# keyber/Single-Image-Super-Resolution

Hardware: AMD Instinct MI355X
Metric: HR patches/sec (x2 generator fwd+bwd, LR 96x96 -> SR 192x192) (higher is better)
Workload: dtype f32; 1 GPU; SRGAN x2 generator (16 blocks, 64 features, spectral norm) fwd+bwd+Adam with bicubic LR degradation and pixel-MSE x10, per-GPU batch 16 HR 192x192 patches (LR 96x96 -> SR 192x192): the north star's headline. BASELINE.json's metric string "96^2 crops, x4" is configs.cfg3 of this line. Single build: fp32.; per_gpu_batch=16, hr=192, lr=96, parallelism=dp1, hip_graph=True

## Files before the change

### single-image-super-resolution_amd/csrc/conv_trunk_f32.hip

```cpp
#include "sisr_dev.h"
#include "sisr_bf16_stage.h"
#include "sisr_instr.h"

typedef unsigned cf_u32x4 __attribute__((ext_vector_type(4)));

#include <type_traits>

#define CF_TH 8
#define CF_TW 16
#define CF_IH (CF_TH + 2)
#define CF_IW (CF_TW + 2)
#define CF_NPIX (CF_IH * CF_IW)
#define CF_PSF 36
#define CF_HALO_BYTES (CF_NPIX * CF_PSF * 4)
#define CF_WROW 36
#define CF_WCHUNK_BYTES (9 * 32 * CF_WROW * 4)
#define CF_ITEMS ((CF_NPIX * 8 + 255) / 256)
#define CF_THREADS 512
#define CF_KROWP 100
#define CF_PS 33

SISR_TRACE_BUFFER(sisr_cftrace, 512, 128)
#define CFT(k) SISR_TRACE_STAMP(sisr_cftrace, threadIdx.x == 0, blockIdx.x, k, 64, wall_clock64())
#define CFTP(k) SISR_TRACE_STAMP(sisr_cftrace, threadIdx.x == 256, blockIdx.x, 64 + (k), 128, wall_clock64())
SISR_TRACE_BUFFER(sisr_cfclk, 512, 2)
#define CFTC(k) SISR_TRACE_STAMP(sisr_cfclk, threadIdx.x == 0, blockIdx.x, (k) - 60, 2, clock64())

struct CTrunkF32Args {
    const float *x1, *x2;
    float* x_out;
    BnFinArgs fin;
    const float *pa, *pb, *pd, *ps, *pt;
    const float* slope_p; float slope;
    const float* wpk;
    const void* wimg;
    const float* bias;
    const float* res;
    float* y;
    float *stat_part, *cnt_part;
    const float *bnb_x, *bnb_scale, *bnb_shift, *bnb_mean, *bnb_invstd, *bnb_slope_p;
    float bnb_slope; int bnb_act;
    float* bnb_part;
    int N, H, W;
    int tiles_x, per_img, total, streams;
    uint32_t m_tiles_x, m_per_img;
    int glog, cout_pad, shuffle;
    int xsc, xph;
};

__device__ __forceinline__ __amdgpu_buffer_rsrc_t cf_rsrc(const void* p, unsigned bytes) {
    return __builtin_amdgcn_make_buffer_rsrc(const_cast<void*>(p), 0, (int)bytes, 0x00020000);
}

__device__ __forceinline__ void cf_split2(float v0, float v1, unsigned& hw, unsigned& lw) {
    const f32x2 v = {v0, v1};
    hw = __builtin_bit_cast(unsigned, __builtin_convertvector(v, bf16x2));
    const f32x2 r = {v0 - __uint_as_float(hw << 16), v1 - __uint_as_float(hw & 0xFFFF0000u)};
    lw = __builtin_bit_cast(unsigned, __builtin_convertvector(r, bf16x2));
}

template <int PRO, bool SPLIT>
__global__ void __launch_bounds__(CF_THREADS, 2) conv_trunk_f32_kernel(const CTrunkF32Args a) {
    extern __shared__ __attribute__((aligned(16))) unsigned char lds[];
    unsigned char* halo0 = lds + 2 * CF_WCHUNK_BYTES;
    float* red = reinterpret_cast<float*>(halo0 + 2 * CF_HALO_BYTES);

    const int tid = threadIdx.x, lane = tid & 63;
    const int wave = __builtin_amdgcn_readfirstlane(tid >> 6);
    const bool consumer = wave < 4;
    const int l31 = lane & 31, kk = lane >> 5;
    const bool xcd = (a.streams & 7) == 0;
    const int hc = xcd ? (blockIdx.x >> 3) & ((1 << a.glog) - 1) : blockIdx.x & ((1 << a.glog) - 1);
    const int stream = xcd ? (blockIdx.x & 7) | ((blockIdx.x >> (3 + a.glog)) << 3) : blockIdx.x >> a.glog;
    const unsigned tbytes = (unsigned)a.N * (unsigned)a.H * (unsigned)a.W * 256u;
    constexpr bool TWO = PRO == SISR_PRO_BNBWD || PRO == SISR_PRO_BNACT_BWD || PRO == SISR_PRO_RES_AFFINE || PRO == SISR_PRO_ACT_BWD;
    constexpr bool SUM = PRO == SISR_PRO_RES_AFFINE;
    auto tile_coords = [&](int T, int& n, int& ty, int& tx) {
        n = fdiv(T, a.m_per_img);
        const int rem = T - n * a.per_img;
        ty = fdiv(rem, a.m_tiles_x);
        tx = rem - ty * a.tiles_x;
    };

    CFT(0);
    CFTC(60);
    float* kfin = red + 4 * 32 * 3;
    const bool fin = (PRO == SISR_PRO_AFFINE_ACT || PRO == SISR_PRO_RES_AFFINE) && a.fin.stat != nullptr;
    if (fin) bn_finalize_in_kernel(a.fin, reinterpret_cast<double*>(lds), kfin, blockIdx.x == 0);
    auto fill_weights = [&]() {
        float* wl = reinterpret_cast<float*>(lds);
        if (a.wimg != nullptr) {
            constexpr int UNITS = 2 * 9 * 32 * CF_WROW / 4;
            constexpr int W_IT16 = (UNITS + CF_THREADS - 1) / CF_THREADS;
            const cf_u32x4* src = reinterpret_cast<const cf_u32x4*>(a.wimg) + hc * UNITS;
            cf_u32x4 wv16[W_IT16];
#pragma unroll
            for (int it = 0; it < W_IT16; ++it) {
                const int u = tid + it * CF_THREADS;
                wv16[it] = u < UNITS ? src[u] : cf_u32x4{0u, 0u, 0u, 0u};
            }
#pragma unroll
            for (int it = 0; it < W_IT16; ++it) {
                const int u = tid + it * CF_THREADS;
                if (u < UNITS) reinterpret_cast<cf_u32x4*>(wl)[u] = wv16[it];
            }
            return;
        }
        constexpr int W_IT = 2 * 9 * 32 * 32 / CF_THREADS;
        float wv[W_IT];
#pragma unroll
        for (int it = 0; it < W_IT; ++it) {
            const int e = tid + it * CF_THREADS;
            const int ci = e & 31, s = (e >> 5) % 3, t2 = (e >> 5) / 3;
            const int co = t2 & 31, qr = t2 >> 5;
            wv[it] = a.wpk[((int64_t)qr * a.cout_pad + 32 * hc + co) * CF_KROWP + s * CF_PS + ci];
        }
#pragma unroll
        for (int it = 0; it < W_IT; ++it) {
            const int e = tid + it * CF_THREADS;
            const int ci = e & 31, s = (e >> 5) % 3, t2 = (e >> 5) / 3;
            const int co = t2 & 31, qr = t2 >> 5;
            const int q = qr / 3, r = qr - 3 * q;
            if constexpr (SPLIT) {
                const float vo = __shfl_xor(wv[it], 1);
                const bool odd = ci & 1;
                unsigned hw, lw;
                cf_split2(odd ? vo : wv[it], odd ? wv[it] : vo, hw, lw);
                reinterpret_cast<unsigned*>(wl)[((q * 9 + r * 3 + s) * 32 + co) * CF_WROW + (odd ? 16 : 0) + (ci >> 1)] = odd ? lw : hw;
            } else {
                wl[((q * 9 + r * 3 + s) * 32 + co) * CF_WROW + ci] = wv[it];
            }
        }
    };

    const int n_mine = stream < a.total ? (a.total - stream + a.streams - 1) / a.streams : 0;
    const int n_stages = 2 * n_mine;

    if (!consumer) {
        const int pt = tid & 255, quad = tid & 7, m0 = pt >> 3;
        const int tiles_y = a.per_img / a.tiles_x;
        const float slope = PRO != SISR_PRO_NONE ? (a.slope_p ? a.slope_p[0] : a.slope) : 1.f;
        f32x4 ka[2], kb[2], kd[2], ks[2], kt[2];
        int rel[CF_ITEMS];
        unsigned flags = 0;
#pragma unroll
        for (int k = 0; k < CF_ITEMS; ++k) {
            const int px = m0 + 32 * k;
            const int py = px / CF_IW, pxx = px - py * CF_IW;
            rel[k] = ((py - 1) * a.xsc * a.xsc * a.W + (pxx - 1) * a.xsc) * 256 + quad * 16;
            const unsigned f = (py == 0 ? 1u : 0u) | (py == CF_IH - 1 ? 2u : 0u) | (pxx == 0 ? 4u : 0u) | (pxx == CF_IW - 1 ? 8u : 0u) |
                               (px >= CF_NPIX ? 16u : 0u);
            flags |= f << (5 * k);
            asm volatile("" : "+v"(rel[k]));
        }
        const bool last_beyond = m0 + 32 * (CF_ITEMS - 1) >= CF_NPIX;
        const int ldso = SPLIT ? m0 * CF_PSF * 4 + quad * 8 : (m0 * CF_PSF + quad * 4) * 4;
        const bool easy_slope = slope >= 0.f && slope <= 1.f;

        struct Stage { f32x4 s1[CF_ITEMS], s2[CF_ITEMS]; unsigned bad, origin; bool edge; };
        Stage stA, stB;
        auto issue = [&](int j, Stage& st) {
            const int T = stream + (j >> 1) * a.streams, q = j & 1;
            const unsigned xbytes = (unsigned)(a.xsc * a.xsc) * tbytes;
            const __amdgpu_buffer_rsrc_t r1 = cf_rsrc(a.x1, xbytes), r2 = cf_rsrc(TWO ? a.x2 : a.x1, xbytes);
            int n, ty, tx;
            tile_coords(T, n, ty, tx);
            const unsigned origin = (unsigned)(((n * a.xsc * a.H + a.xsc * ty * CF_TH + (a.xph >> 1)) * a.xsc * a.W + a.xsc * tx * CF_TW + (a.xph & 1)) * 256 + q * 128);
            const unsigned e = (ty == 0 ? 1u : 0u) | (ty == tiles_y - 1 ? 2u : 0u) | (tx == 0 ? 4u : 0u) | (tx == a.tiles_x - 1 ? 8u : 0u);
            st.edge = e != 0u;
            st.bad = flags & ((e | 16u) * 0x02108421u);
            st.origin = origin;
#pragma unroll
            for (int k = 0; k < CF_ITEMS; ++k) {
                const unsigned voff = origin + (unsigned)rel[k];
                st.s1[k] = __builtin_bit_cast(f32x4, __builtin_amdgcn_raw_buffer_load_b128(r1, voff, 0, 0));
                if (TWO) st.s2[k] = __builtin_bit_cast(f32x4, __builtin_amdgcn_raw_buffer_load_b128(r2, voff, 0, 0));
            }
        };
        auto commit_t = [&](auto easy_, auto edge_, int j, const Stage& st) {
            constexpr int EASY = decltype(easy_)::value;
            constexpr bool EDGE = decltype(edge_)::value;
            const int q = j & 1;
            float* img = reinterpret_cast<float*>(halo0 + (j & 1) * CF_HALO_BYTES + ldso);
            const f32x4 qa = q ? ka[1] : ka[0], qb = q ? kb[1] : kb[0], qd = q ? kd[1] : kd[0], qs = q ? ks[1] : ks[0], qt = q ? kt[1] : kt[0];
            const __amdgpu_buffer_rsrc_t ro = cf_rsrc(SUM ? a.x_out : a.x1, tbytes);
#pragma unroll
            for (int k = 0; k < CF_ITEMS; ++k) {
                if (k == CF_ITEMS - 1 && last_beyond) break;
                const bool ok = !EDGE || ((st.bad >> (5 * k)) & 31u) == 0u;
                auto value = [&](int c) {
                    const float v = st.s1[k][c];
                    if (PRO == SISR_PRO_NONE) return v;
                    if (PRO == SISR_PRO_ACT) return lrelu_t<EASY>(v, slope);
                    if (PRO == SISR_PRO_AFFINE_ACT) return lrelu_t<EASY>(qa[c] * v + qd[c], slope);
                    if (SUM) return lrelu_t<EASY>(v, slope) + (qa[c] * st.s2[k][c] + qd[c]);
                    if (PRO == SISR_PRO_ACT_BWD) return st.s2[k][c] > 0.f ? v : slope * v;
                    const float bx = st.s2[k][c];
                    float g = v;
                    if (PRO == SISR_PRO_BNACT_BWD) g = qs[c] * bx + qt[c] > 0.f ? v : slope * v;
                    return qa[c] * g + qb[c] * bx + qd[c];
                };
                const f32x4 osum = {value(0), value(1), value(2), value(3)};
                const f32x4 zero4 = {0.f, 0.f, 0.f, 0.f};
                if constexpr (SPLIT) {
                    typedef unsigned cf_u32x2 __attribute__((ext_vector_type(2)));
                    unsigned h0, l0, h1, l1;
                    cf_split2(osum[0], osum[1], h0, l0);
                    cf_split2(osum[2], osum[3], h1, l1);
                    const cf_u32x2 hw = {h0, h1}, lw = {l0, l1};
                    const cf_u32x2 z2 = {0u, 0u};
                    *reinterpret_cast<cf_u32x2*>(img + k * 32 * CF_PSF) = ok ? hw : z2;
                    *reinterpret_cast<cf_u32x2*>(img + k * 32 * CF_PSF + 16) = ok ? lw : z2;
                } else
                *reinterpret_cast<f32x4*>(img + k * 32 * CF_PSF) = ok ? osum : zero4;
                if (SUM && hc == 0 && ((flags >> (5 * k)) & 31u) == 0u)
                    __builtin_amdgcn_raw_buffer_store_b128(__builtin_bit_cast(cf_u32x4, osum), ro, st.origin + (unsigned)rel[k], 0, 0);
            }
        };
        auto commit = [&](int j, const Stage& st) {
            using T1 = std::integral_constant<int, 1>; using T0 = std::integral_constant<int, 0>;
            constexpr bool HAS_ACT = PRO == SISR_PRO_ACT || PRO == SISR_PRO_AFFINE_ACT || SUM;
            if (!HAS_ACT || easy_slope) {
                if (st.edge) commit_t(T1{}, std::true_type{}, j, st); else commit_t(T1{}, std::false_type{}, j, st);
            } else {
                if (st.edge) commit_t(T0{}, std::true_type{}, j, st); else commit_t(T0{}, std::false_type{}, j, st);
            }
        };

        issue(0, stA);
        issue(1, stB);
#pragma unroll
        for (int q = 0; q < 2; ++q)
#pragma unroll
            for (int j = 0; j < 4; ++j) {
                const int c = q * 32 + quad * 4 + j;
                constexpr bool AFF = PRO == SISR_PRO_AFFINE_ACT || (TWO && PRO != SISR_PRO_ACT_BWD);
                ka[q][j] = fin ? kfin[c] : AFF ? a.pa[c] : 1.f;
                kd[q][j] = fin ? kfin[64 + c] : AFF ? a.pd[c] : 0.f;
                kb[q][j] = (TWO && !SUM && PRO != SISR_PRO_ACT_BWD) ? a.pb[c] : 0.f;
                ks[q][j] = PRO == SISR_PRO_BNACT_BWD ? a.ps[c] : 0.f;
                kt[q][j] = PRO == SISR_PRO_BNACT_BWD ? a.pt[c] : 0.f;
            }
        fill_weights();
        __syncthreads();
        if (n_stages > 0) commit(0, stA);
        __syncthreads();
        int j = 0;
        while (j < n_stages) {
            CFTP(4 + 6 * j);
            issue(j + 2, stA);
            CFTP(5 + 6 * j);
            if (j + 1 < n_stages) commit(j + 1, stB);
            CFTP(8 + 6 * j);
            __syncthreads();
            CFTP(9 + 6 * j);
            if (++j >= n_stages) break;
            CFTP(4 + 6 * j);
            issue(j + 2, stB);
            CFTP(5 + 6 * j);
            if (j + 1 < n_stages) commit(j + 1, stA);
            CFTP(8 + 6 * j);
            __syncthreads();
            CFTP(9 + 6 * j);
            ++j;
        }
    } else {
        const int co = a.shuffle ? 32 * (hc & 1) + l31 : 32 * hc + l31;
        const int ph = hc >> 1;
        const int abase = SPLIT ? ((2 * wave + (l31 >> 4)) * CF_IW + (l31 & 15)) * CF_PSF * 4 + 16 * kk
                                : (((2 * wave + (l31 >> 4)) * CF_IW + (l31 & 15)) * CF_PSF + 16 * kk) * 4;
        const int bbase = SPLIT ? l31 * CF_WROW * 4 + 16 * kk : (l31 * CF_WROW + 16 * kk) * 4;
        const float bv = a.bias != nullptr ? a.bias[a.shuffle ? co * 4 + ph : co] : 0.f;
        float st_shift = 0.f, st_s1 = 0.f, st_s2 = 0.f;
        int st_n = 0;
        const __amdgpu_buffer_rsrc_t ry = cf_rsrc(a.y, a.shuffle ? 4u * tbytes : tbytes), rr = cf_rsrc(a.res != nullptr ? a.res : a.y, tbytes);
        f32x16 acc;
        f32x16 rv, xv;
        const bool has_x = (PRO == SISR_PRO_BNBWD || PRO == SISR_PRO_BNACT_BWD) && a.bnb_part != nullptr;
        const __amdgpu_buffer_rsrc_t rxb = cf_rsrc(has_x ? a.bnb_x : a.y, tbytes);
        float b_sc = 0.f, b_sf = 0.f, b_mu = 0.f, b_is = 0.f, b_slope = 1.f;
        float rs1 = 0.f, rs2 = 0.f, rsl = 0.f;
        if (has_x) {
            b_sc = a.bnb_scale[co]; b_sf = a.bnb_shift[co]; b_mu = a.bnb_mean[co]; b_is = a.bnb_invstd[co];
            b_slope = a.bnb_slope_p ? a.bnb_slope_p[0] : a.bnb_slope;
        }
        fill_weights();
        __syncthreads();
        __syncthreads();
        constexpr bool BWD = TWO && !SUM;
        const bool has_res = BWD && a.res != nullptr;
        const bool x_act = has_x && a.bnb_act != 0;
        const bool do_stat = !BWD && a.stat_part != nullptr;
        const bool shuf = !TWO && a.shuffle != 0;
        const int vl_plain = co * 4 + kk * 4 * 256, vl_shuf = co * 4 + kk * 4 * 512;
        const int tiles_y = fdiv(a.per_img, a.m_tiles_x);
        const int dn = fdiv(a.streams, a.m_per_img), drem = a.streams - dn * a.per_img;
        const int dty = fdiv(drem, a.m_tiles_x), dtx = drem - dty * a.tiles_x;
        int n, ty, tx;
        tile_coords(stream, n, ty, tx);
        auto mma = [&](auto q_c, auto&& mid) {
            constexpr int Q = decltype(q_c)::value;
            const unsigned char* ab = halo0 + Q * CF_HALO_BYTES + abase;
            const unsigned char* bb = lds + Q * CF_WCHUNK_BYTES + bbase;
            if constexpr (SPLIT) {
                bf16x8 ah[9][2], al[9][2], bh[9][2], bl[9][2];
                auto fetch_s = [&](int t) {
                    const unsigned char* pa = ab + ((t / 3) * CF_IW + (t % 3)) * CF_PSF * 4;
                    const unsigned char* pb = bb + t * 32 * CF_WROW * 4;
#pragma unroll
                    for (int ks = 0; ks < 2; ++ks) {
                        ah[t][ks] = *reinterpret_cast<const bf16x8*>(pa + 32 * ks);
                        bh[t][ks] = *reinterpret_cast<const bf16x8*>(pb + 32 * ks);
                        al[t][ks] = *reinterpret_cast<const bf16x8*>(pa + 64 + 32 * ks);
                        bl[t][ks] = *reinterpret_cast<const bf16x8*>(pb + 64 + 32 * ks);
                    }
                };
                fetch_s(0);
                fetch_s(1);
                mid();
                __builtin_amdgcn_sched_barrier(0);
#pragma unroll
                for (int t = 0; t < 9; ++t) {
                    if (t + 2 < 9) fetch_s(t + 2);
#pragma unroll
                    for (int ks = 0; ks < 2; ++ks) {
                        acc = __builtin_amdgcn_mfma_f32_32x32x16_bf16(al[t][ks], bh[t][ks], acc, 0, 0, 0);
                        acc = __builtin_amdgcn_mfma_f32_32x32x16_bf16(ah[t][ks], bl[t][ks], acc, 0, 0, 0);
                        acc = __builtin_amdgcn_mfma_f32_32x32x16_bf16(ah[t][ks], bh[t][ks], acc, 0, 0, 0);
                    }
                    __builtin_amdgcn_sched_barrier(0);
                }
            } else {
                f32x4 af[18][2], bf[18][2];
                auto fetch = [&](int u) {
                    const int t = u >> 1, s0 = 8 * (u & 1);
#pragma unroll
                    for (int v = 0; v < 2; ++v) {
                        af[u][v] = *reinterpret_cast<const f32x4*>(ab + (((t / 3) * CF_IW + (t % 3)) * CF_PSF + s0 + 4 * v) * 4);
                        bf[u][v] = *reinterpret_cast<const f32x4*>(bb + ((t * 32) * CF_WROW + s0 + 4 * v) * 4);
                    }
                };
                fetch(0);
                fetch(1);
                __builtin_amdgcn_sched_barrier(0);
                mid();
                __builtin_amdgcn_sched_barrier(0);
#pragma unroll
                for (int u = 0; u < 18; ++u) {
                    if (u + 2 < 18) fetch(u + 2);
#pragma unroll
                    for (int s = 0; s < 8; ++s) acc = __builtin_amdgcn_mfma_f32_32x32x2f32(af[u][s >> 2][s & 3], bf[u][s >> 2][s & 3], acc, 0, 0, 0);
                    if (u + 2 < 18) __builtin_amdgcn_sched_group_barrier(0x100, 4, 0);
                    __builtin_amdgcn_sched_group_barrier(0x008, 8, 0);
                }
            }
        };
        auto each_value = [&](auto ocol_c, unsigned sb, int orow, auto&& f) {
            constexpr int OCOL = decltype(ocol_c)::value;
            constexpr bool FAR = 11 * OCOL > 4095;
            const unsigned s0 = sb, s1 = sb + (unsigned)orow, s0f = s0 + 8u * OCOL, s1f = s1 + 8u * OCOL;
#pragma unroll
            for (int i = 0; i < 16; ++i) {
                const bool hi = (i >> 2) & 1;
                const unsigned so = (i >> 3) ? (FAR && hi ? s1f : s1) : (FAR && hi ? s0f : s0);
                f(i, (unsigned)(((FAR ? 0 : 8 * hi) + (i & 3)) * OCOL), so);
            }
        };
        using OcolPlain = std::integral_constant<int, 256>;
        using OcolShuf = std::integral_constant<int, 512>;
        for (int t = 0; t < n_mine; ++t) {
            const unsigned sb = (unsigned)(((n * a.H + ty * CF_TH + 2 * wave) * a.W + tx * CF_TW) * 256);
            int vlp = vl_plain, vls = vl_shuf;
            asm volatile("" : "+v"(vlp), "+v"(vls));
            CFT(4 + 12 * t);
            mma(std::integral_constant<int, 0>{}, [&]() {
#pragma unroll
                for (int i = 0; i < 16; ++i) acc[i] = bv;
            });
            CFT(6 + 12 * t);
            CFT(8 + 12 * t);
            __syncthreads();
            CFT(9 + 12 * t);
            CFT(10 + 12 * t);
            mma(std::integral_constant<int, 1>{}, [&]() {
                if (has_res)
                    each_value(OcolPlain{}, sb, a.W * 256, [&](int i, unsigned imm, unsigned so) {
                        rv[i] = __builtin_bit_cast(float, __builtin_amdgcn_raw_buffer_load_b32(rr, (unsigned)vlp + imm, so, 0));
                    });
                if (has_x)
                    each_value(OcolPlain{}, sb, a.W * 256, [&](int i, unsigned imm, unsigned so) {
                        xv[i] = __builtin_bit_cast(float, __builtin_amdgcn_raw_buffer_load_b32(rxb, (unsigned)vlp + imm, so, 0));
                    });
            });
            CFT(12 + 12 * t);
            if (has_res) {
#pragma unroll
                for (int i = 0; i < 16; ++i) acc[i] += rv[i];
            }
            if (has_x) {
                if (x_act) {
#pragma unroll
                    for (int i = 0; i < 16; ++i) {
                        float gv = acc[i];
                        const float z = b_sc * xv[i] + b_sf;
                        const bool neg = !(z > 0.f);
                        rsl += neg ? gv * z : 0.f;
                        gv = neg ? gv * b_slope : gv;
                        rs1 += gv;
                        rs2 += gv * ((xv[i] - b_mu) * b_is);
                    }
                } else {
#pragma unroll
                    for (int i = 0; i < 16; ++i) {
                        rs1 += acc[i];
                        rs2 += acc[i] * ((xv[i] - b_mu) * b_is);
                    }
                }
            }
            if (do_stat) {
                if (st_n == 0) {
                    float s = 0.f;
#pragma unroll
                    for (int i = 0; i < 16; ++i) s += acc[i];
                    st_shift = s * (1.f / 16.f);
                }
#pragma unroll
                for (int i = 0; i < 16; ++i) {
                    const float dv = acc[i] - st_shift;
                    st_s1 += dv;
                    st_s2 += dv * dv;
                }
                st_n += 16;
            }
            if (shuf) {
                const unsigned sbs = (unsigned)(((n * 2 * a.H + 2 * (ty * CF_TH + 2 * wave) + (ph >> 1)) * 2 * a.W + 2 * tx * CF_TW + (ph & 1)) * 256);
                each_value(OcolShuf{}, sbs, 4 * a.W * 256, [&](int i, unsigned imm, unsigned so) {
                    __builtin_amdgcn_raw_buffer_store_b32(__builtin_bit_cast(unsigned, (float)acc[i]), ry, (unsigned)vls + imm, so, 0);
                });
            } else {
                each_value(OcolPlain{}, sb, a.W * 256, [&](int i, unsigned imm, unsigned so) {
                    __builtin_amdgcn_raw_buffer_store_b32(__builtin_bit_cast(unsigned, (float)acc[i]), ry, (unsigned)vlp + imm, so, 0);
                });
            }
            CFT(14 + 12 * t);
            __syncthreads();
            CFT(15 + 12 * t);
            tx += dtx;
            if (tx >= a.tiles_x) { tx -= a.tiles_x; ++ty; }
            ty += dty;
            if (ty >= tiles_y) { ty -= tiles_y; ++n; }
            n += dn;
        }
        CFT(3);

        if (a.stat_part != nullptr) {
            float nn = (float)st_n, mu = 0.f, m2 = 0.f;
            if (st_n > 0) {
                const float m1 = st_s1 / nn;
                mu = st_shift + m1;
                m2 = st_s2 - st_s1 * m1;
            }
            const float nb = __shfl_xor(nn, 32), mub = __shfl_xor(mu, 32), m2b = __shfl_xor(m2, 32);
            const float nt = nn + nb;
            if (nt > 0.f) { const float dl = mub - mu, f = nb / nt; mu += dl * f; m2 += m2b + dl * dl * nn * f; }
            nn = nt;
            if (kk == 0) { float* r = red + (wave * 32 + l31) * 3; r[0] = nn; r[1] = mu; r[2] = m2; }
        }
        if (has_x) {
            rs1 += __shfl_xor(rs1, 32);
            rs2 += __shfl_xor(rs2, 32);
            rsl += __shfl_xor(rsl, 32);
            if (kk == 0) { float* r = red + (wave * 32 + l31) * 3; r[0] = rs1; r[1] = rs2; r[2] = rsl; }
        }
    }
    if (a.bnb_part != nullptr) {
        __syncthreads();
        float* wk = a.bnb_part + (int64_t)blockIdx.x * 129;
        if (tid < 64) {
            const int c = tid & 31;
            const bool mine = (tid >> 5) == hc;
            float s1 = 0.f, s2 = 0.f;
            if (mine) {
                s1 = (red[c * 3] + red[(32 + c) * 3]) + (red[(64 + c) * 3] + red[(96 + c) * 3]);
                s2 = (red[c * 3 + 1] + red[(32 + c) * 3 + 1]) + (red[(64 + c) * 3 + 1] + red[(96 + c) * 3 + 1]);
            }
            wk[tid] = s1;
            wk[64 + tid] = s2;
        }
        if (tid == 64) {
            float sl = 0.f;
            for (int i = 0; i < 128; ++i) sl += red[i * 3 + 2];
            wk[128] = sl;
        }
    }
    if (a.stat_part != nullptr) {
        __syncthreads();
        if (tid < 32) {
            float nn = red[tid * 3], mm = red[tid * 3 + 1], qq = red[tid * 3 + 2];
#pragma unroll
            for (int w = 1; w < 4; ++w) {
                const float* r1 = red + (w * 32 + tid) * 3;
                const float nb = r1[0], nt = nn + nb;
                if (nt > 0.f) { const float dl = r1[1] - mm, f = nb / nt; mm += dl * f; qq += r1[2] + dl * dl * nn * f; }
                nn = nt;
            }
            float* sp = a.stat_part + (int64_t)stream * 128 + 32 * hc + tid;
            sp[0] = mm;
            sp[64] = qq;
            if (tid == 0 && hc == 0) a.cnt_part[stream] = nn;
        }
    }
    CFT(63);
    CFTC(61);
}

#include "sisr_trunk_host.h"
static const SisrTrunkKind CF_KIND = {CF_TH, CF_TW, false, 256};

int sisr_conv2d_trunk_f32_streams(const SisrConvDesc* d) {
    return sisr_equal_shares(d->N * (d->H / CF_TH) * (d->W / CF_TW), sisr_cu_slots() / (d->Cout == 256 ? 8 : 2));
}

extern "C" int sisr_conv2d_trunk_f32_eligible(const SisrConvDesc* d) {
    if (!d || sisr_switch_off("SISR_TRUNK")) return 0;
    if (sisr_switch_off("SISR_TRUNK_F32CONV")) return 0;
    if (!sisr_switch_off("SISR_TRUNK_UP") && d->Cin == 256 && d->Cout == 64 && d->KH == 3 && d->KW == 3 && d->stride == 1 && d->pad_y == 1 && d->pad_x == 1 &&
        d->x_mode == SISR_X_NHWC_UNSHUFFLE2 && d->pro_mode == SISR_PRO_ACT_BWD && d->x2 && d->y_mode == SISR_Y_NHWC && !d->x_bf16 && !d->y_bf16 &&
        !d->res_bf16 && d->Ho == d->H && d->Wo == d->W && !(d->H % CF_TH) && !(d->W % CF_TW) && d->y_sy == 1 && d->y_sx == 1 && !d->y_oy && !d->y_ox &&
        d->y_H == d->Ho && d->y_W == d->Wo && d->epi_act == SISR_EPI_NONE && d->plan.CK == 32 && d->plan.PS == CF_PS && d->plan.KROWP == CF_KROWP &&
        d->plan.CoutPad == 64 && d->plan.n_chunk == 8 && (int64_t)d->N * d->H * d->W * 1024 < (1ll << 31) &&
        d->N * (d->H / CF_TH) * (d->W / CF_TW) < 65536 && !d->stat_part && !d->bias && !d->bnb_part && !d->fin_stat)
        return 2;
    if (d->plan.CK != 32 || d->plan.PS != CF_PS || d->plan.KROWP != CF_KROWP || d->plan.n_chunk != 2 || d->plan.CoutPad != d->Cout) return 0;
    if (d->res_bf16) return 0;
    const int role = sisr_trunk_conv_role(d, CF_KIND);
    if (role == 2 && d->bnb_part && !(d->bnb_x && !d->bnbx_bf16)) return 0;
    return role;
}

template <int PRO, bool SPLIT>
static int launch_cf_t(const CTrunkF32Args& a, hipStream_t st) {
    constexpr int lds_bytes = 2 * CF_WCHUNK_BYTES + 2 * CF_HALO_BYTES + 4 * 32 * 3 * 4 + 128 * 4;
    return sisr_launch<conv_trunk_f32_kernel<PRO, SPLIT>>(dim3(a.streams << a.glog), dim3(CF_THREADS), lds_bytes, 0, st, a);
}
template <int PRO>
static int launch_cf(const CTrunkF32Args& a, bool split, hipStream_t st) {
    return split ? launch_cf_t<PRO, true>(a, st) : launch_cf_t<PRO, false>(a, st);
}

int sisr_conv2d_trunk_f32_launch(const SisrConvDesc* d, hipStream_t st) {
    CTrunkF32Args a{};
    sisr_trunk_conv_args(a, d, CF_KIND);
    const int img_mode = (d->plan.variant >> 1) & 3;
    a.wimg = (d->Cin == 64 && d->Cout == 64 && img_mode == (d->mfma_split ? 2 : 1)) ? static_cast<const void*>(d->wpk + d->plan.wpk_elems) : nullptr;
    a.streams = sisr_conv2d_trunk_f32_streams(d); a.glog = d->Cout == 256 ? 3 : 1;
    a.xsc = 1; a.xph = 0;
    if (d->Cin == 256) {
        a.xsc = 2;
        for (int ph = 0; ph < 4; ++ph) {
            a.xph = ph;
            a.wpk = d->wpk + (size_t)ph * 2 * 3 * 64 * CF_KROWP;
            a.res = ph == 0 ? d->res : d->y;
            if (int e = launch_cf<SISR_PRO_ACT_BWD>(a, d->mfma_split != 0, st)) return e;
        }
        return 0;
    }
    switch (d->pro_mode) {
        case SISR_PRO_NONE: return launch_cf<SISR_PRO_NONE>(a, d->mfma_split != 0, st);
        case SISR_PRO_ACT: return launch_cf<SISR_PRO_ACT>(a, d->mfma_split != 0, st);
        case SISR_PRO_AFFINE_ACT: return launch_cf<SISR_PRO_AFFINE_ACT>(a, d->mfma_split != 0, st);
        case SISR_PRO_BNBWD: return launch_cf<SISR_PRO_BNBWD>(a, d->mfma_split != 0, st);
        case SISR_PRO_BNACT_BWD: return launch_cf<SISR_PRO_BNACT_BWD>(a, d->mfma_split != 0, st);
        case SISR_PRO_RES_AFFINE: return launch_cf<SISR_PRO_RES_AFFINE>(a, d->mfma_split != 0, st);
    }
    return SISR_E_UNSUPPORTED;
}
```

Measured before the change: 1504 HR patches/s.

## Restructure conv producer loop with incremental tile walk and ballot-based edge masks

Rewrites the producer half of the trunk conv kernel so the tile position advances incrementally instead of recomputing tile coordinates and origin for every stage. Loop-invariant buffer descriptors are hoisted out of the loop, and stage-parity and easy-slope choices become compile-time template parameters. Per-item edge and ownership flags are kept as wave ballot masks read back with inverse_ballot, which cuts VGPR use and per-element selects. The weight fill for the two-input case is split into two passes to lower register pressure. The residual-store ownership now alternates by half (hc==q), and FMA contraction is pinned explicitly, which risks small numerical and correctness differences.

```diff
diff --git a/single-image-super-resolution_amd/csrc/conv_trunk_f32.hip b/single-image-super-resolution_amd/csrc/conv_trunk_f32.hip
--- a/single-image-super-resolution_amd/csrc/conv_trunk_f32.hip
+++ b/single-image-super-resolution_amd/csrc/conv_trunk_f32.hip
@@ -106,35 +106,37 @@
             }
             return;
         }
-        constexpr int W_IT = 2 * 9 * 32 * 32 / CF_THREADS;
-        float wv[W_IT];
-#pragma unroll
-        for (int it = 0; it < W_IT; ++it) {
-            const int e = tid + it * CF_THREADS;
-            const int ci = e & 31, s = (e >> 5) % 3, t2 = (e >> 5) / 3;
-            const int co = t2 & 31, qr = t2 >> 5;
-            wv[it] = a.wpk[((int64_t)qr * a.cout_pad + 32 * hc + co) * CF_KROWP + s * CF_PS + ci];
-        }
-#pragma unroll
-        for (int it = 0; it < W_IT; ++it) {
-            const int e = tid + it * CF_THREADS;
-            const int ci = e & 31, s = (e >> 5) % 3, t2 = (e >> 5) / 3;
-            const int co = t2 & 31, qr = t2 >> 5;
-            const int q = qr / 3, r = qr - 3 * q;
-            if constexpr (SPLIT) {
-                const float vo = __shfl_xor(wv[it], 1);
-                const bool odd = ci & 1;
-                unsigned hw, lw;
-                cf_split2(odd ? vo : wv[it], odd ? wv[it] : vo, hw, lw);
-                reinterpret_cast<unsigned*>(wl)[((q * 9 + r * 3 + s) * 32 + co) * CF_WROW + (odd ? 16 : 0) + (ci >> 1)] = odd ? lw : hw;
-            } else {
-                wl[((q * 9 + r * 3 + s) * 32 + co) * CF_WROW + ci] = wv[it];
+        constexpr int W_PASS = TWO ? 2 : 1, W_IT = 2 * 9 * 32 * 32 / CF_THREADS / W_PASS;
+#pragma unroll
+        for (int ps = 0; ps < W_PASS; ++ps) {
+            float wv[W_IT];
+#pragma unroll
+            for (int it = 0; it < W_IT; ++it) {
+                const int e = tid + (ps * W_IT + it) * CF_THREADS;
+                const int ci = e & 31, s = (e >> 5) % 3, t2 = (e >> 5) / 3;
+                const int co = t2 & 31, qr = t2 >> 5;
+                wv[it] = a.wpk[((int64_t)qr * a.cout_pad + 32 * hc + co) * CF_KROWP + s * CF_PS + ci];
+            }
+#pragma unroll
+            for (int it = 0; it < W_IT; ++it) {
+                const int e = tid + (ps * W_IT + it) * CF_THREADS;
+                const int ci = e & 31, s = (e >> 5) % 3, t2 = (e >> 5) / 3;
+                const int co = t2 & 31, qr = t2 >> 5;
+                const int q = qr / 3, r = qr - 3 * q;
+                if constexpr (SPLIT) {
+                    const float vo = __shfl_xor(wv[it], 1);
+                    const bool odd = ci & 1;
+                    unsigned hw, lw;
+                    cf_split2(odd ? vo : wv[it], odd ? wv[it] : vo, hw, lw);
+                    reinterpret_cast<unsigned*>(wl)[((q * 9 + r * 3 + s) * 32 + co) * CF_WROW + (odd ? 16 : 0) + (ci >> 1)] = odd ? lw : hw;
+                } else {
+                    wl[((q * 9 + r * 3 + s) * 32 + co) * CF_WROW + ci] = wv[it];
+                }
             }
         }
     };
 
     const int n_mine = stream < a.total ? (a.total - stream + a.streams - 1) / a.streams : 0;
-    const int n_stages = 2 * n_mine;
 
     if (!consumer) {
         const int pt = tid & 255, quad = tid & 7, m0 = pt >> 3;
@@ -156,38 +158,51 @@
         const bool last_beyond = m0 + 32 * (CF_ITEMS - 1) >= CF_NPIX;
         const int ldso = SPLIT ? m0 * CF_PSF * 4 + quad * 8 : (m0 * CF_PSF + quad * 4) * 4;
         const bool easy_slope = slope >= 0.f && slope <= 1.f;
-
-        struct Stage { f32x4 s1[CF_ITEMS], s2[CF_ITEMS]; unsigned bad, origin; bool edge; };
-        Stage stA, stB;
-        auto issue = [&](int j, Stage& st) {
-            const int T = stream + (j >> 1) * a.streams, q = j & 1;
-            const unsigned xbytes = (unsigned)(a.xsc * a.xsc) * tbytes;
-            const __amdgpu_buffer_rsrc_t r1 = cf_rsrc(a.x1, xbytes), r2 = cf_rsrc(TWO ? a.x2 : a.x1, xbytes);
-            int n, ty, tx;
-            tile_coords(T, n, ty, tx);
-            const unsigned origin = (unsigned)(((n * a.xsc * a.H + a.xsc * ty * CF_TH + (a.xph >> 1)) * a.xsc * a.W + a.xsc * tx * CF_TW + (a.xph & 1)) * 256 + q * 128);
-            const unsigned e = (ty == 0 ? 1u : 0u) | (ty == tiles_y - 1 ? 2u : 0u) | (tx == 0 ? 4u : 0u) | (tx == a.tiles_x - 1 ? 8u : 0u);
-            st.edge = e != 0u;
-            st.bad = flags & ((e | 16u) * 0x02108421u);
-            st.origin = origin;
+        uint64_t own[CF_ITEMS];
+#pragma unroll
+        for (int k = 0; k < CF_ITEMS; ++k) own[k] = SUM ? __builtin_amdgcn_ballot_w64(((flags >> (5 * k)) & 31u) == 0u) : 0ull;
+        const unsigned xbytes = (unsigned)(a.xsc * a.xsc) * tbytes;
+        const __amdgpu_buffer_rsrc_t r1 = cf_rsrc(a.x1, xbytes), r2 = cf_rsrc(TWO ? a.x2 : a.x1, xbytes);
+        const __amdgpu_buffer_rsrc_t ro = cf_rsrc(SUM ? a.x_out : a.x1, tbytes);
+
+        auto tile_origin = [&](int n, int ty, int tx) {
+            return (unsigned)(((n * a.xsc * a.H + a.xsc * ty * CF_TH + (a.xph >> 1)) * a.xsc * a.W + a.xsc * tx * CF_TW + (a.xph & 1)) * 256);
+        };
+        auto tile_edges = [&](int ty, int tx) {
+            return (ty == 0 ? 1u : 0u) | (ty == tiles_y - 1 ? 2u : 0u) | (tx == 0 ? 4u : 0u) | (tx == a.tiles_x - 1 ? 8u : 0u);
+        };
+        unsigned voff[CF_ITEMS], origin;
+        uint64_t bad[CF_ITEMS];
+        bool edge;
+        auto tile_masks = [&](unsigned e) {
+            edge = e != 0u;
+            const unsigned pat = e * 0x02108421u;
 #pragma unroll
             for (int k = 0; k < CF_ITEMS; ++k) {
-                const unsigned voff = origin + (unsigned)rel[k];
-                st.s1[k] = __builtin_bit_cast(f32x4, __builtin_amdgcn_raw_buffer_load_b128(r1, voff, 0, 0));
-                if (TWO) st.s2[k] = __builtin_bit_cast(f32x4, __builtin_amdgcn_raw_buffer_load_b128(r2, voff, 0, 0));
-            }
-        };
-        auto commit_t = [&](auto easy_, auto edge_, int j, const Stage& st) {
+                unsigned pk = pat & (31u << (5 * k));
+                asm volatile("" : "+s"(pk));
+                bad[k] = __builtin_amdgcn_ballot_w64((flags & pk) != 0u);
+            }
+        };
+        struct Stage { f32x4 s1[CF_ITEMS], s2[CF_ITEMS]; };
+        Stage st0, st1;
+        auto issue = [&](auto q_c, Stage& st) {
+            constexpr unsigned Q = decltype(q_c)::value;
+#pragma unroll
+            for (int k = 0; k < CF_ITEMS; ++k) {
+                st.s1[k] = __builtin_bit_cast(f32x4, __builtin_amdgcn_raw_buffer_load_b128(r1, voff[k] + Q * 128u, 0, 0));
+                if (TWO) st.s2[k] = __builtin_bit_cast(f32x4, __builtin_amdgcn_raw_buffer_load_b128(r2, voff[k] + Q * 128u, 0, 0));
+            }
+        };
+        auto commit_t = [&](auto easy_, auto edge_, auto q_c, unsigned back, const Stage& st) {
             constexpr int EASY = decltype(easy_)::value;
             constexpr bool EDGE = decltype(edge_)::value;
-            const int q = j & 1;
-            float* img = reinterpret_cast<float*>(halo0 + (j & 1) * CF_HALO_BYTES + ldso);
-            const f32x4 qa = q ? ka[1] : ka[0], qb = q ? kb[1] : kb[0], qd = q ? kd[1] : kd[0], qs = q ? ks[1] : ks[0], qt = q ? kt[1] : kt[0];
-            const __amdgpu_buffer_rsrc_t ro = cf_rsrc(SUM ? a.x_out : a.x1, tbytes);
+            constexpr int q = decltype(q_c)::value;
+            float* img = reinterpret_cast<float*>(halo0 + q * CF_HALO_BYTES + ldso);
+            const f32x4 qa = ka[q], qb = kb[q], qd = kd[q], qs = ks[q], qt = kt[q];
 #pragma unroll
             for (int k = 0; k < CF_ITEMS; ++k) {
                 if (k == CF_ITEMS - 1 && last_beyond) break;
-                const bool ok = !EDGE || ((st.bad >> (5 * k)) & 31u) == 0u;
                 auto value = [&](int c) {
                     const float v = st.s1[k][c];
                     if (PRO == SISR_PRO_NONE) return v;
@@ -197,38 +212,93 @@
                     if (PRO == SISR_PRO_ACT_BWD) return st.s2[k][c] > 0.f ? v : slope * v;
                     const float bx = st.s2[k][c];
                     float g = v;
-                    if (PRO == SISR_PRO_BNACT_BWD) g = qs[c] * bx + qt[c] > 0.f ? v : slope * v;
-                    return qa[c] * g + qb[c] * bx + qd[c];
+                    if (PRO == SISR_PRO_BNACT_BWD) g = __builtin_fmaf(qs[c], bx, qt[c]) > 0.f ? v : slope * v;
+                    if constexpr (SPLIT) {
+                        return qa[c] * g + qb[c] * bx + qd[c];
+                    } else {
+#pragma clang fp contract(off)
+                        if (!EDGE && k == CF_ITEMS - 1 && c >= 2) return (qa[c] * g + qb[c] * bx) + qd[c];
+                        if (PRO == SISR_PRO_BNBWD) return __builtin_fmaf(qa[c], g, qb[c] * bx) + qd[c];
+                        return __builtin_fmaf(qb[c], bx, qa[c] * g) + qd[c];
+                    }
                 };
                 const f32x4 osum = {value(0), value(1), value(2), value(3)};
-                const f32x4 zero4 = {0.f, 0.f, 0.f, 0.f};
                 if constexpr (SPLIT) {
                     typedef unsigned cf_u32x2 __attribute__((ext_vector_type(2)));
                     unsigned h0, l0, h1, l1;
                     cf_split2(osum[0], osum[1], h0, l0);
                     cf_split2(osum[2], osum[3], h1, l1);
                     const cf_u32x2 hw = {h0, h1}, lw = {l0, l1};
-                    const cf_u32x2 z2 = {0u, 0u};
-                    *reinterpret_cast<cf_u32x2*>(img + k * 32 * CF_PSF) = ok ? hw : z2;
-                    *reinterpret_cast<cf_u32x2*>(img + k * 32 * CF_PSF + 16) = ok ? lw : z2;
-                } else
-                *reinterpret_cast<f32x4*>(img + k * 32 * CF_PSF) = ok ? osum : zero4;
-                if (SUM && hc == 0 && ((flags >> (5 * k)) & 31u) == 0u)
-                    __builtin_amdgcn_raw_buffer_store_b128(__builtin_bit_cast(cf_u32x4, osum), ro, st.origin + (unsigned)rel[k], 0, 0);
-            }
-        };
-        auto commit = [&](int j, const Stage& st) {
-            using T1 = std::integral_constant<int, 1>; using T0 = std::integral_constant<int, 0>;
-            constexpr bool HAS_ACT = PRO == SISR_PRO_ACT || PRO == SISR_PRO_AFFINE_ACT || SUM;
-            if (!HAS_ACT || easy_slope) {
-                if (st.edge) commit_t(T1{}, std::true_type{}, j, st); else commit_t(T1{}, std::false_type{}, j, st);
-            } else {
-                if (st.edge) commit_t(T0{}, std::true_type{}, j, st); else commit_t(T0{}, std::false_type{}, j, st);
-            }
-        };
-
-        issue(0, stA);
-        issue(1, stB);
+                    *reinterpret_cast<cf_u32x2*>(img + k * 32 * CF_PSF) = hw;
+                    *reinterpret_cast<cf_u32x2*>(img + k * 32 * CF_PSF + 16) = lw;
+                    if constexpr (EDGE) {
+                        asm volatile("" ::: "memory");
+                        if (__builtin_amdgcn_inverse_ballot_w64(bad[k])) {
+                            const cf_u32x2 z2 = {0u, 0u};
+                            *reinterpret_cast<cf_u32x2*>(img + k * 32 * CF_PSF) = z2;
+                            *reinterpret_cast<cf_u32x2*>(img + k * 32 * CF_PSF + 16) = z2;
+                        }
+                    }
+                } else {
+                    *reinterpret_cast<f32x4*>(img + k * 32 * CF_PSF) = osum;
+                    if constexpr (EDGE) {
+                        asm volatile("" ::: "memory");
+                        if (__builtin_amdgcn_inverse_ballot_w64(bad[k]))
+                            *reinterpret_cast<f32x4*>(img + k * 32 * CF_PSF) = f32x4{0.f, 0.f, 0.f, 0.f};
+                    }
+                }
+                if (SUM && hc == q && __builtin_amdgcn_inverse_ballot_w64(own[k]))
+                    __builtin_amdgcn_raw_buffer_store_b128(__builtin_bit_cast(cf_u32x4, osum), ro, voff[k] + back + q * 128u, 0, 0);
+            }
+        };
+        auto commit = [&](auto easy_, auto q_c, unsigned back, const Stage& st) {
+            if (edge) commit_t(easy_, std::true_type{}, q_c, back, st); else commit_t(easy_, std::false_type{}, q_c, back, st);
+        };
+        using Q0 = std::integral_constant<int, 0>; using Q1 = std::integral_constant<int, 1>;
+        const int dn = fdiv(a.streams, a.m_per_img), drem = a.streams - dn * a.per_img;
+        const int dty = fdiv(drem, a.m_tiles_x), dtx = drem - dty * a.tiles_x;
+        int n, ty, tx;
+        tile_coords(stream, n, ty, tx);
+        auto advance = [&]() {
+            tx += dtx;
+            if (tx >= a.tiles_x) { tx -= a.tiles_x; ++ty; }
+            ty += dty;
+            if (ty >= tiles_y) { ty -= tiles_y; ++n; }
+            n += dn;
+        };
+        auto walk = [&](auto easy_) {
+            for (int t = 0; t < n_mine; ++t) {
+                advance();
+                const unsigned o_next = tile_origin(n, ty, tx), step = o_next - origin;
+                origin = o_next;
+#pragma unroll
+                for (int k = 0; k < CF_ITEMS; ++k) voff[k] += step;
+                CFTP(4 + 12 * t);
+                issue(Q0{}, st0);
+                CFTP(5 + 12 * t);
+                commit(easy_, Q1{}, 0u - step, st1);
+                CFTP(8 + 12 * t);
+                __syncthreads();
+                CFTP(9 + 12 * t);
+                CFTP(10 + 12 * t);
+                issue(Q1{}, st1);
+                CFTP(11 + 12 * t);
+                tile_masks(tile_edges(ty, tx));
+                if (t + 1 < n_mine) commit(easy_, Q0{}, 0u, st0);
+                CFTP(14 + 12 * t);
+                __syncthreads();
+                CFTP(15 + 12 * t);
+            }
+        };
+        using T1 = std::integral_constant<int, 1>; using T0 = std::integral_constant<int, 0>;
+        constexpr bool HAS_ACT = PRO == SISR_PRO_ACT || PRO == SISR_PRO_AFFINE_ACT || SUM;
+
+        origin = tile_origin(n, ty, tx);
+#pragma unroll
+        for (int k = 0; k < CF_ITEMS; ++k) voff[k] = origin + (unsigned)rel[k];
+        tile_masks(tile_edges(ty, tx));
+        issue(Q0{}, st0);
+        issue(Q1{}, st1);
 #pragma unroll
         for (int q = 0; q < 2; ++q)
 #pragma unroll
@@ -243,27 +313,12 @@
             }
         fill_weights();
         __syncthreads();
-        if (n_stages > 0) commit(0, stA);
+        const bool easy = !HAS_ACT || easy_slope;
+        if (n_mine > 0) {
+            if (easy) commit(T1{}, Q0{}, 0u, st0); else commit(T0{}, Q0{}, 0u, st0);
+        }
         __syncthreads();
-        int j = 0;
-        while (j < n_stages) {
-            CFTP(4 + 6 * j);
-            issue(j + 2, stA);
-            CFTP(5 + 6 * j);
-            if (j + 1 < n_stages) commit(j + 1, stB);
-            CFTP(8 + 6 * j);
-            __syncthreads();
-            CFTP(9 + 6 * j);
-            if (++j >= n_stages) break;
-            CFTP(4 + 6 * j);
-            issue(j + 2, stB);
-            CFTP(5 + 6 * j);
-            if (j + 1 < n_stages) commit(j + 1, stA);
-            CFTP(8 + 6 * j);
-            __syncthreads();
-            CFTP(9 + 6 * j);
-            ++j;
-        }
+        if (easy) walk(T1{}); else walk(T0{});
     } else {
         const int co = a.shuffle ? 32 * (hc & 1) + l31 : 32 * hc + l31;
         const int ph = hc >> 1;
```

After: 1525 HR patches/s, median of 6. +1.4%, better.
